# Tarekbouamer/Image-Retrieval-for-Image-Based-Localization

Measured on AMD Instinct MI355X. Metric: images/sec extract + queries/sec 1M-desc kNN, ResNet50-GeM 1024×768, higher is better.
Workload: dtype fp16

## Files before the change

### image-retrieval-for-image-based-localization_amd/cirtorch/_engine.py

```python

import contextlib
import ctypes
import os
import threading

import torch

PKG_DIR = os.path.dirname(os.path.dirname(os.path.abspath(__file__)))
LIB_PATH = os.environ.get("RR_LIB", os.path.join(PKG_DIR, "librr.so"))

RR_F32, RR_BF16, RR_F16, RR_I8 = 0, 1, 2, 3
RR_ACT_IDENTITY, RR_ACT_LEAKY = 0, 1
RR_POOL_GEM, RR_POOL_MAC, RR_POOL_SPOC = 0, 1, 2
RR_CONV_AFFINE, RR_CONV_RESIDUAL, RR_CONV_PERM32 = 1, 2, 4
RR_NHWC, RR_NCHW = 0, 1
RR_MATCH_NN, RR_MATCH_MNN, RR_MATCH_SNN, RR_MATCH_SMNN = 0, 1, 2, 3
RR_RESP_HARRIS, RR_RESP_GFTT, RR_RESP_HESSIAN, RR_RESP_DOG = 0, 1, 2, 3
RR_EPI_SAMPSON, RR_EPI_SYMMETRICAL = 0, 1
TUNE_KEYS = ("GEMM_CONFIG", "GEMM_STAGES", "GEMM_WIDE", "GEMM_ASTAT", "GEMM_XCD_MAP", "STREAM_1X1", "CONV3X3",
             "GRID_CUS", "GEMM8", "KNN_FUSED", "CONV3_PIPE", "STEM", "STREAM_XCD", "CONV3S", "WRES", "PAIR_MID",
             "WRES_RING")
globals().update(("RR_TUNE_" + name, key) for key, name in enumerate(TUNE_KEYS))
TUNE_SIZE_KEYS = {"PATCHNET_CHUNK": 32}
globals().update(("RR_TUNE_" + name, key) for name, key in TUNE_SIZE_KEYS.items())
# ... 10 lines not shown


class LaunchInfo(ctypes.Structure):
    _fields_ = [("kernel", ctypes.c_char * 32), ("variant", ctypes.c_char * 48), ("grid", ctypes.c_uint),
                ("block", ctypes.c_uint), ("nslices", ctypes.c_int), ("xmap", ctypes.c_int), ("launches", ctypes.c_int)]


class Region(ctypes.Structure):
    _fields_ = [(n, ctypes.c_uint16) for n in ("y0", "x0", "h", "w")]


_vp, _i, _ll, _f, _d, _sz = ctypes.c_void_p, ctypes.c_int, ctypes.c_longlong, ctypes.c_float, ctypes.c_double, ctypes.c_size_t
_SIGS = {
    "rr_version": ([], _i),
    "rr_build_info": ([], ctypes.c_char_p),
    "rr_last_error": ([], ctypes.c_char_p),
    "rr_device_arch": ([ctypes.c_char_p, _i], _i),
    "rr_image_to_nhwc": ([_vp, _i, _i, _i, _i, ctypes.POINTER(_f), ctypes.POINTER(_f), _i, _vp, _i, _i, _vp], _i),
    "rr_conv2d_fused": ([_vp, _vp, _vp, _vp, _vp, _vp, ctypes.POINTER(ConvDesc), _i, _i, _vp], _i),
    "rr_conv1x1_pair": ([_vp, _ll, _i, _vp, _vp, _vp, _i, _vp, _vp, _vp, _vp, _vp, _i, _f, _vp, _vp, _vp, _i, _i, _f,
                         _vp, _vp, _i, _vp], _i),
    "rr_conv3x3_pair": ([_vp, _i, _i, _i, _vp, _vp, _vp, _i, _f, _vp, _vp, _vp, _i, _f, _vp, _vp, _vp, _vp, _vp, _vp, _vp, _vp, _i, _f,
                         _vp, _vp, _vp, _i, _i, _f, _vp, _vp, _vp, _i, _vp], _i),
    "rr_pack_conv_weights": ([_vp, _i, _i, _i, _i, _i, _i, _i, _vp, _i, _vp], _i),
    "rr_stem_pack_weights": ([_vp, _i, _i, _i, _i, _vp, _i, _vp], _i),
    "rr_stem_conv_pool": ([_vp, _i, _i, _i, ctypes.POINTER(_f), ctypes.POINTER(_f), _i, _vp, _vp, _vp, _i, _f, _vp,
                           _i, _i, _i, _vp], _i),
    "rr_stem_conv_pool_u8": ([_vp, _i, _i, _i, ctypes.POINTER(_f), ctypes.POINTER(_f), _i, _vp, _vp, _vp, _i, _f,
                              _vp, _i, _i, _i, _vp], _i),
    "rr_image_to_nhwc_ragged": ([_vp, _vp, _i, _i, _i, _i, _i, ctypes.POINTER(_f), ctypes.POINTER(_f), _i, _vp, _i,
                                 _i, _vp], _i),
    "rr_stem_conv_pool_ragged": ([_vp, _vp, _i, _i, _i, _i, ctypes.POINTER(_f), ctypes.POINTER(_f), _i, _vp, _vp, _vp,
                                  _i, _f, _vp, _i, _i, _i, _vp], _i),
    "rr_pad_images": ([_vp, _vp, _i, _i, _i, _i, _i, _vp, _vp, _vp], _i),
    "rr_maxpool2d": ([_vp, _i, _i, _i, _i, _i, _i, _i, _vp, _i, _i, _i, _vp], _i),
    "rr_resize_bilinear": ([_vp, _i, _i, _i, _vp, _i, _i, _d, _d, _vp], _i),
    "rr_global_pool": ([_vp, _i, _i, _i, _i, _i, _f, _f, _vp, _i, _vp], _i),
    "rr_global_pool_pdev": ([_vp, _i, _i, _i, _i, _i, _f, _vp, _f, _vp, _i, _vp], _i),
    "rr_region_pool": ([_vp, _i, _i, _i, _i, ctypes.POINTER(Region), _i, _i, _f, _vp, _i, _f, _vp, _i, _vp], _i),
    "rr_region_aggregate": ([_vp, _i, _i, _i, _i, _f, _vp, _vp], _i),
    "rr_l2n_rows": ([_vp, _i, _i, _f, _vp, _vp], _i),
    "rr_linear_rows": ([_vp, _i, _i, _vp, _vp, _i, _vp, _vp], _i),
    "rr_head_workspace_bytes": ([_i, _i], _sz),
    "rr_whiten_workspace_bytes": ([_i, _i], _sz),
    "rr_whitenapply": ([_vp, _i, _i, _vp, _vp, _i, _vp, _vp, _sz, _vp], _i),
    "rr_head_l2n_whiten_l2n": ([_vp, _i, _i, _vp, _vp, _i, _f, _vp, _vp, _vp], _i),
# ... 192 lines not shown
```

### image-retrieval-for-image-based-localization_amd/cirtorch/_ops.py

```python

import ctypes
import os

import numpy as np
import torch

from . import _engine as E


def _st():
    return E.stream_ptr()


def _workspace(nbytes, device):
    return torch.empty(max(int(nbytes), 256), dtype=torch.uint8, device=device)


def image_to_nhwc(img, c_pad, dtype, mean=None, std=None):
    E.require_gpu(img)
    img = img.contiguous().float()
    n, c, h, w = img.shape
    out = torch.empty((n, h, w, c_pad), dtype=dtype, device=img.device)
    do = mean is not None
    m = (ctypes.c_float * 4)(*(list(mean) + [0.0] * (4 - c))[:4]) if do else (ctypes.c_float * 4)()
# ... 59 lines not shown
    E.require_gpu(x, w3, residual, w1)
    n, h, w, c = x.shape
    c_mid = w3.shape[0]
    y, z = _pair_out(out, (n, h, w, c_mid), (n, h, w, c_out), x.dtype, x.device)
    assert x.is_contiguous()
    if residual is not None:
        assert residual.shape == y.shape and residual.dtype == x.dtype and residual.is_contiguous()
        xp = wp = sp = hp = None
    else:
        xp, wp, sp, hp = proj
        E.require_gpu(xp, wp, sp, hp)
        assert xp.shape == x.shape and xp.dtype == x.dtype and xp.is_contiguous()
    E.check(E.lib().rr_conv1x1_pair(E.ptr(x), n * h * w, c, E.ptr(w3), E.ptr(scale3), E.ptr(shift3), c_mid,
                                    E.ptr(residual), E.ptr(xp), E.ptr(wp), E.ptr(sp), E.ptr(hp),
                                    E.RR_ACT_LEAKY if leaky3 else E.RR_ACT_IDENTITY, float(slope3),
                                    E.ptr(w1), E.ptr(scale1), E.ptr(shift1), c_out,
                                    E.RR_ACT_LEAKY if leaky1 else E.RR_ACT_IDENTITY, float(slope1), E.ptr(y), E.ptr(z),
                                    E.dtype_code(x.dtype), _st()), "rr_conv1x1_pair")
    return y, z


def conv3x3_pair(t1, w33, scale2, shift2, leaky2, slope2, w3, scale3, shift3, residual, leaky3, slope3,
                 w1, scale1, shift1, c_out, leaky1, slope1, proj=None, dynamic=None, conv1=None,
                 out=None):
    E.require_gpu(t1, w33, w3, residual, w1)
    n, h, w, c = t1.shape
    assert c == 64 and t1.is_contiguous() and tuple(w33.shape) == (64, 576) and tuple(w3.shape) == (256, 64)
    assert tuple(w1.shape) == (c_out, 256)
    y, z = _pair_out(out, (n, h, w, 256), (n, h, w, c_out), t1.dtype, t1.device)
    if residual is not None:
        assert residual.shape == y.shape and residual.dtype == t1.dtype and residual.is_contiguous()
        xp = wp = sp = hp = None
    else:
        xp, wp, sp, hp = proj
        E.require_gpu(xp, wp, sp, hp)
        assert tuple(xp.shape) == (n, h, w, 64) and xp.dtype == t1.dtype and xp.is_contiguous()
    act = lambda leaky: E.RR_ACT_LEAKY if leaky else E.RR_ACT_IDENTITY
    if dynamic is None:
        dynamic = os.environ.get("RR_C3PAIR_QUEUE", "1") != "0"
    queue = torch.zeros(8, dtype=torch.int32, device=t1.device) if dynamic else None
    w0, s0, h0, leaky0, slope0 = conv1 if conv1 is not None else (None, None, None, False, 0.0)
    if conv1 is not None:
        E.require_gpu(w0, s0, h0)
        assert proj is not None and tuple(w0.shape) == (64, 64)
    E.check(E.lib().rr_conv3x3_pair(E.ptr(t1), n, h, w, E.ptr(w0), E.ptr(s0), E.ptr(h0), act(leaky0), float(slope0),
                                    E.ptr(w33), E.ptr(scale2), E.ptr(shift2), act(leaky2),
                                    float(slope2), E.ptr(w3), E.ptr(scale3), E.ptr(shift3), E.ptr(residual),
                                    E.ptr(xp), E.ptr(wp), E.ptr(sp), E.ptr(hp), act(leaky3), float(slope3),
                                    E.ptr(w1), E.ptr(scale1), E.ptr(shift1), c_out, act(leaky1), float(slope1),
                                    E.ptr(y), E.ptr(z), E.ptr(queue), E.dtype_code(t1.dtype), _st()),
            "rr_conv3x3_pair")
    return y, z


def maxpool2d(x, k=3, stride=2, pad=1):
    E.require_gpu(x)
    n, h, w, c = x.shape
    ho = (h + 2 * pad - k) // stride + 1
    wo = (w + 2 * pad - k) // stride + 1
    y = torch.empty((n, ho, wo, c), dtype=x.dtype, device=x.device)
    E.check(E.lib().rr_maxpool2d(E.ptr(x), n, h, w, c, k, stride, pad, E.ptr(y), ho, wo, E.dtype_code(x.dtype),
                                 _st()), "rr_maxpool2d")
    return y


def pack_stem_weights(weight, dtype=torch.bfloat16):
    E.require_gpu(weight)
    w = weight.detach().float().contiguous()
    co, ci, kh, kw = w.shape
    out = torch.empty((co, 448), dtype=dtype, device=w.device)
    E.check(E.lib().rr_stem_pack_weights(E.ptr(w), co, ci, kh, kw, E.ptr(out), E.dtype_code(dtype), _st()),
            "rr_stem_pack_weights")
    return out

# ... 1221 lines not shown
```

### image-retrieval-for-image-based-localization_amd/cirtorch/backbones/misc.py

```python

from collections import OrderedDict

import torch
import torch.nn as nn

from .. import _ops
from ..modules.abn import ABN


class ConvStep:
    __slots__ = ("w", "kh", "kw", "stride", "pad", "c_out", "scale", "shift", "leaky", "slope", "perm")


def make_step(conv, bn, dtype, cin_pad=None, leaky_override=None):
    st = ConvStep()
    co, ci, kh, kw = conv.weight.shape
    cin_pad = cin_pad or ci
    st.perm = co % 32 == 0
    st.w = _ops.pack_conv_weights(conv.weight, cin_pad, dtype, perm32=st.perm)
    st.kh, st.kw = kh, kw
    st.stride = conv.stride[0]
    st.pad = conv.padding[0]
    st.c_out = co
    st.scale, st.shift = bn.folded()
    st.leaky, st.slope = bn.slope()
    if leaky_override is not None:
        st.leaky = leaky_override
    return st


def run_step(t, st, residual=None, out=None):
    return _ops.conv2d_fused(t, st.w, st.kh, st.kw, st.stride, st.pad, st.c_out, st.scale, st.shift,
                             residual=residual, leaky=st.leaky, slope=st.slope, perm32=st.perm, out=out)


class ResidualBlock(nn.Module):
    def __init__(self, in_channels, channels, stride=1, dilation=1, groups=1, norm_act=ABN, dropout=None):
        super().__init__()
        if len(channels) != 2 and len(channels) != 3:
            raise ValueError("channels must contain either two or three values")
        if len(channels) == 2 and groups != 1:
            raise ValueError("groups > 1 are only valid if len(channels) == 3")
        if groups != 1 or dilation != 1:
            raise NotImplementedError("grouped / dilated residual blocks are out of scope")
        self.is_bottleneck = len(channels) == 3
        self.stride = stride
# ... 64 lines not shown
```

### image-retrieval-for-image-based-localization_amd/cirtorch/backbones/resnet.py

```python

import os
import sys
from collections import OrderedDict
from functools import partial

import torch
import torch.nn as nn
import torch.nn.functional as F

from .. import _ops
from ..modules.abn import ABN
from .misc import ResidualBlock, make_step, run_step

CONV_PARAMS = ["weight"]
BN_PARAMS = ["weight", "bias", "running_mean", "running_var"]

_PRECISIONS = {"bf16": torch.bfloat16, "fp32": torch.float32, "float32": torch.float32, "bfloat16": torch.bfloat16,
               "fp16": torch.float16, "float16": torch.float16}


def try_index(scalar_or_list, i):
    try:
        return scalar_or_list[i]
    except TypeError:
# ... 94 lines not shown
        self._plan = None
        return super()._load_from_state_dict(*args, **kwargs)

    def stem_cin(self):
        return 4 if self.engine_dtype == torch.float32 else 8

    def _step(self, conv, bn, cin_pad=None, leaky_override=None):
        return make_step(conv, bn, self.engine_dtype, cin_pad=cin_pad, leaky_override=leaky_override)

    def _build_plan(self):
        dev = self.mod1.conv1.weight.device
        if dev.type != "cuda":
            raise RuntimeError("the MI355X engine runs on the GPU: call .cuda() on the model first")
        plan = {"stem": self._step(self.mod1.conv1, self.mod1.bn1, cin_pad=self.stem_cin()), "mods": []}
        plan["stem_fused"] = None
        if self.engine_dtype in (torch.bfloat16, torch.float16) and tuple(self.mod1.conv1.weight.shape) == (64, 3, 7, 7) \
                and hasattr(self.mod1, "pool1") and os.environ.get("RR_STEM_FUSED", "1") != "0":
            plan["stem_fused"] = _ops.pack_stem_weights(self.mod1.conv1.weight, self.engine_dtype)
        for mod_id in range(4):
            mod = getattr(self, "mod%d" % (mod_id + 2))
            blocks = []
            for blk in mod.children():
                blocks.append(blk.engine_plan(self.engine_dtype))
            plan["mods"].append(blocks)
        self._plan = plan
        return plan

    @staticmethod
    def _conv(t, st, residual=None, out=None):
        return run_step(t, st, residual, out)

    def _stem(self, plan, x, mean, std):
        if isinstance(x, (list, tuple)):
            live = [t for t in x if t is not None]
            if not live:
                raise ValueError("at least one image of the batch must be non-None")
            h = max(int(t.shape[-2]) for t in live)
            w = max(int(t.shape[-1]) for t in live)
            st = plan["stem"]
            if plan["stem_fused"] is not None:
                return _ops.stem_conv_pool_ragged(x, h, w, plan["stem_fused"], st.scale, st.shift, leaky=st.leaky,
                                                  slope=st.slope, mean=mean, std=std)
            t = _ops.image_to_nhwc_ragged(x, h, w, self.stem_cin(), self.engine_dtype, mean, std)
            return _ops.maxpool2d(self._conv(t, st), 3, 2, 1)
        if x.dtype == torch.uint8 and plan["stem_fused"] is None:
            x = _ops.pixels_to_unit(x)
        if plan["stem_fused"] is not None:
            st = plan["stem"]
            return _ops.stem_conv_pool(x, plan["stem_fused"], st.scale, st.shift, leaky=st.leaky, slope=st.slope,
                                       mean=mean, std=std)
        t = _ops.image_to_nhwc(x, self.stem_cin(), self.engine_dtype, mean, std)
        t = self._conv(t, plan["stem"])
        return _ops.maxpool2d(t, 3, 2, 1)

    def _blocks(self, t, flat, i0, i1, outs, pending=None):
        for i in range(i0, i1):
            mod_id, steps, proj = flat[i]
            nxt = flat[i + 1][1][0] if i + 1 < i1 else None
            pair = self._pairable(steps[-1], nxt)
            fuse_proj = pair and proj is not None and self._proj_fusable(proj)
            res = t if proj is None else (None if fuse_proj else self._conv(t, proj))
            block = pair and self._c3pairable(t, steps, nxt, fuse_proj)
            conv1 = block and fuse_proj and pending is None and self._conv1_fusable(t, steps[0])
            y = t
            for j, st in enumerate(steps[:-2] if block else steps[:-1]):
                if conv1:
                    break
                y = pending if (j == 0 and pending is not None) else self._conv(y, st)
            pending = None
            if block:
                mid, last = steps[-2], steps[-1]
                c1 = steps[0]
                t, pending = _ops.conv3x3_pair(y, mid.w, mid.scale, mid.shift, mid.leaky, mid.slope,
                                               last.w, last.scale, last.shift, res, last.leaky, last.slope,
                                               nxt.w, nxt.scale, nxt.shift, nxt.c_out, nxt.leaky, nxt.slope,
                                               proj=(t, proj.w, proj.scale, proj.shift) if fuse_proj else None,
                                               conv1=(c1.w, c1.scale, c1.shift, c1.leaky, c1.slope) if conv1 else None)
            elif pair:
                last = steps[-1]
                t, pending = _ops.conv1x1_pair(y, last.w, last.scale, last.shift, res, last.leaky, last.slope,
                                               nxt.w, nxt.scale, nxt.shift, nxt.c_out, nxt.leaky, nxt.slope,
                                               proj=(t, proj.w, proj.scale, proj.shift) if fuse_proj else None)
            else:
                t = self._conv(y, steps[-1], residual=res)
            if outs is not None and (i + 1 == len(flat) or flat[i + 1][0] != mod_id):
                outs["mod%d" % (mod_id + 2)] = t
        return t, pending

    def forward(self, x, normalize=None):
        plan = self._plan or self._build_plan()
        mean, std = normalize if normalize is not None else (None, None)
        outs = OrderedDict()
        flat = [(mod_id, steps, proj) for mod_id, blocks in enumerate(plan["mods"]) for steps, proj in blocks]
        t = self._stem(plan, x, mean, std)
        outs["mod1"] = t
        self._blocks(t, flat, 0, len(flat), outs)
        return OrderedDict((k, v.permute(0, 3, 1, 2)) for k, v in outs.items())

    @staticmethod
    def _proj_fusable(proj):
        return (proj.kh == 1 and proj.stride == 1 and proj.pad == 0 and proj.perm and proj.c_out == 256
                and proj.w.shape[1] == 64 and not proj.leaky)

    @staticmethod
    def _c3pairable(t, steps, nxt, fuse_proj):
        if len(steps) != 3 or os.environ.get("RR_C3PAIR", "1") == "0":
            return False
        mid, last = steps[1], steps[2]
        n, h, w, c = t.shape
        return (mid.kh == 3 and mid.kw == 3 and mid.stride == 1 and mid.pad == 1 and mid.perm and mid.c_out == 64
                and tuple(mid.w.shape) == (64, 576) and last.c_out == 256 and last.w.shape[1] == 64
                and nxt.c_out in ((64,) if fuse_proj else (64, 128)) and h % 4 == 0 and w % 32 == 0
                and n * h * w * 64 * 2 < 2 ** 31)

    @staticmethod
    def _conv1_fusable(t, st):
        return (os.environ.get("RR_C3PAIR_CONV1", "0") == "1" and st.kh == 1 and st.kw == 1 and st.stride == 1
                and st.pad == 0 and st.perm and st.c_out == 64 and tuple(st.w.shape) == (64, 64) and t.shape[-1] == 64)

    def _pairable(self, last, nxt):
# ... 26 lines not shown
```

### image-retrieval-for-image-based-localization_amd/cirtorch/models/GF_net.py

```python

import os
from collections import OrderedDict

import numpy as np
import torch
import torch.nn as nn

from .. import _ops
from ..algos.GF_algo import globalFeatureAlgo
from ..backbones import resnet as _resnet
from ..modules.heads.global_head import globalHead
from ..modules.pools import POOLING_LAYERS
from ..utils.parallel import PackedSequence

from ..modules.utils import OUTPUT_DIM


class Normalize:

    def __init__(self, rgb_mean=(0.485, 0.456, 0.406), rgb_std=(0.229, 0.224, 0.225)):
        self.rgb_mean = list(rgb_mean)
        self.rgb_std = list(rgb_std)


# ... 3 lines not shown
        self.augment = augment
        self.body = body
        self.ret_algo = ret_algo
        self.ret_head = ret_head
        self.meta = {}

    def _prepare_pyramid_inputs(self, img, scales):
        out = []
        for scale in scales:
            if scale == 1:
                out.append(img)
            else:
                out.append(PackedSequence([_ops.resize_bilinear(im, scale) for im in img]))
        return out

    def _normalizer(self):
        a = self.augment
        if a is None:
            return None
        if hasattr(a, "rgb_mean") and hasattr(a, "rgb_std"):
            return (list(a.rgb_mean), list(a.rgb_std))
        raise NotImplementedError("only normalising augment objects (rgb_mean/rgb_std) are supported at eval time")

    @property
    def pool(self):
        return self.ret_head.pool

    def meta_repr(self):
        tmp = "  (meta): dict( \n"
        for k in ("architecture", "local_whitening", "pooling", "regional", "whitening", "outputdim", "mean", "std"):
            if k in self.meta:
                tmp += "     %s: %s\n" % (k, self.meta[k])
        tmp += "  )\n"
        return tmp

    def forward(self, img=None, positive_img=None, negative_img=None, scales=[1], do_augmentaton=False,
                do_loss=False, do_prediction=True, **varargs):
        if do_loss:
            raise NotImplementedError("training (tuple loss) is out of scope for the MI355X engine")
        if isinstance(img, torch.Tensor) and img.dim() == 4 and len(scales) == 1:
            x = self.body(img, normalize=self._normalizer())
            ret_pred = self.ret_algo.inference(self.ret_head, x, [img.shape[-2:]] * img.shape[0]) \
                if do_prediction else None
            return OrderedDict([("ret_loss", None)]), OrderedDict([("ret_pred", ret_pred)])
        if isinstance(img, torch.Tensor) and img.dim() == 4:
            preds = []
            for scale in scales:
                if scale == 1:
                    xs = img
                else:
                    xf = _ops.pixels_to_unit(img) if img.dtype == torch.uint8 else img
                    xs = _ops.resize_bilinear(xf, scale)
                _, pred = self.forward(img=xs, scales=[1], do_prediction=True, do_loss=False)
                preds.append(pred["ret_pred"].unsqueeze(0))
            pred = torch.cat(preds, dim=0).permute(1, 2, 0)
            pred = nn.functional.avg_pool1d(pred, kernel_size=len(scales)).squeeze(-1)
            return OrderedDict([("ret_loss", None)]), OrderedDict([("ret_pred", pred)])
        if isinstance(img, torch.Tensor):
            if img.dtype == torch.uint8 and len(scales) > 1:
                img = _ops.pixels_to_unit(img)
            img = PackedSequence(list(img)) if img.dim() == 4 else PackedSequence([img])
        if len(scales) > 1:
            if img.dtype == torch.uint8:
                img = PackedSequence([_ops.pixels_to_unit(t) if t is not None else None for t in img])
            preds = []
            for im in self._prepare_pyramid_inputs(img, scales):
                _, pred = self.forward(img=im, scales=[1], do_prediction=True, do_loss=False)
                preds.append(pred["ret_pred"].unsqueeze(0))
            pred = torch.cat(preds, dim=0).permute(1, 2, 0)
            pred = nn.functional.avg_pool1d(pred, kernel_size=len(scales)).squeeze(-1)
            return OrderedDict([("ret_loss", None)]), OrderedDict([("ret_pred", pred)])

        images = list(img)
        x = self.body(images, normalize=self._normalizer())
        valid_size = [tuple(t.shape[-2:]) if t is not None else (0, 0) for t in images]
        if do_prediction:
            ret_pred = self.ret_algo.inference(self.ret_head, x, valid_size)
        else:
            ret_pred = None
        return OrderedDict([("ret_loss", None)]), OrderedDict([("ret_pred", ret_pred)])

    def extract(self, images, scales=(1,)):
        if not isinstance(images, torch.Tensor):
            images = PackedSequence(list(images))
        with torch.no_grad():
            _, pred = self.forward(img=images, scales=list(scales))
        return pred["ret_pred"]


def make_net(architecture="resnet50", pooling="gem", whitening=True, mean=None, std=None, precision="bf16",
             p=3.0, regional=False, regional_whitening=True, L=3):
    body = _resnet.__dict__[architecture](precision=precision)
    dim = OUTPUT_DIM[architecture]
    pname = {"gem": "GeM", "mac": "MAC", "spoc": "SPoC", "gemmp": "GeMmp"}[pooling.lower()]
    params = {"p": p, "eps": 1e-6} if pname in ("GeM", "GeMmp") else {}
    if regional:
        if pname == "GeMmp":
# ... 326 lines not shown
```

### image-retrieval-for-image-based-localization_amd/csrc/rr_c3pair.hip

```cpp
#include "rr_internal.h"
#include "rr_ldsdma.h"
#include "rr_epilogue.h"
#include "rr_tilewalk.h"

#ifndef C3P_IG2
#define C3P_IG2 1
#endif

namespace rr {

namespace {

template <int K>
__device__ __forceinline__ int cwswz(int row, int chunk) {
    const int f = K == 64 ? ((row >> 1) & 7) : (row & 15);
    return row * (K * 2) + ((chunk ^ f) << 4);
}

}

struct C3PairArgs {
    const bf16_t* t1;
    const bf16_t* w0;
    const float *s0, *h0;
    const bf16_t* w33;
    const float *s33, *h33;
    const bf16_t* w3;
    const float *s3, *h3;
    const bf16_t* res;
    const bf16_t* xp;
    const bf16_t* wp;
    const float *sp, *hp;
    const bf16_t* w1;
    const float *s1, *h1;
    bf16_t* y;
    bf16_t* z;
    int* queue;
    int n, h, w;
    int act2, act3, act1, act0;
    float slope2, slope3, slope1, slope0;
};

namespace {

template <int C1, bool PROJ, typename HT, bool CONV1 = false>
__global__ void __launch_bounds__(512, 1) k_c3pair(C3PairArgs a, int tiles_w, int tiles_hw, int ntiles) {
    static_assert(!CONV1 || PROJ, "conv1 in the launch: the stage's first block only");
    constexpr int TH = 4, TW = 32, TP = TH * TW, PITCH = 40;
    constexpr int NSLOT = (TH + 2) * PITCH, NP = NSLOT / 8;
    constexpr int PCW = TW + 2;
    constexpr int FN = 4;
    constexpr int K3 = 64, C3 = 256, NK3 = K3 / 32, NR3 = C3 / 32, NF1 = C1 / 16, NK1 = C3 / 32;
    static_assert(NSLOT % 8 == 0 && PITCH % 8 == 0, "row-invariant patch swizzle");
    __shared__ __attribute__((aligned(1024))) char sPatch[NSLOT * 128];
    __shared__ __attribute__((aligned(16))) char sT2[TP * 128];
    __shared__ __attribute__((aligned(16))) char sW3[C3 * K3 * 2];
    __shared__ __attribute__((aligned(16))) char sW1[C1 * C3 * 2];
    __shared__ __attribute__((aligned(16))) char sWp[PROJ ? C3 * K3 * 2 : 16];
    __shared__ __attribute__((aligned(16))) float sS3[C3], sH3[C3], sS1[C1], sH1[C1], sS2[64], sH2[64];
    __shared__ __attribute__((aligned(16))) float sSp[PROJ ? C3 : 4], sHp[PROJ ? C3 : 4];
    __shared__ __attribute__((aligned(16))) char sW0[CONV1 ? 64 * 64 * 2 : 16];
    __shared__ __attribute__((aligned(16))) float sS0[CONV1 ? 64 : 4], sH0[CONV1 ? 64 : 4];
    __shared__ int sTile[4];

    const int tid = threadIdx.x, lane = tid & 63;
    const int wave = __builtin_amdgcn_readfirstlane(tid >> 6);
    const bool role3 = wave < 4;
    const int r16 = lane & 15, kq = lane >> 4, lrow = lane >> 3, lch = lane & 7;
    const int H = a.h, W = a.w;

// ... 154 lines not shown
            sh[r] = sH2[c + r];
        }
        const bool leaky2 = a.act2 == RR_ACT_LEAKY;
#pragma unroll
        for (int j = 0; j < FN; ++j) {
            const int p = wpx * (TP / 2) + j * 16 + r16;
            float v[8];
            RR_BN_PAIR(acc[0][j], acc[1][j], sc, sh, v);
            if (leaky2) RR_LEAKY(8, v, a.slope2);
            uint4 o;
            RR_PACK8(HT, o, v);
            *reinterpret_cast<uint4*>(sT2 + p * 128 + (((4 * wc + kq) ^ (p & 7)) << 4)) = o;
        }
    };

    const int pw = wave - 4;
    const bool leaky3 = a.act3 == RR_ACT_LEAKY, leaky1 = a.act1 == RR_ACT_LEAKY;
    constexpr int NRQ = PROJ ? NK3 : NR3;
    auto strip_pixel = [&](int t, int k) __attribute__((always_inline)) {
        int img, oh0, ow0;
        tile_org(t, img, oh0, ow0);
        return ((long long)img * H + oh0 + (k >> 1)) * W + ow0 + (k & 1) * 16 + r16;
    };
    auto load_rq = [&](uint4 (&dst)[NRQ], long long p) __attribute__((always_inline)) {
        if constexpr (PROJ) {
            const bf16_t* ps = a.xp + p * K3 + 8 * kq;
#pragma unroll
            for (int kk = 0; kk < NK3; ++kk) dst[kk] = ld16_once(ps + kk * 32);
        } else {
            const bf16_t* rs = a.res + p * C3 + 8 * kq;
#pragma unroll
            for (int i2 = 0; i2 < NR3; ++i2) dst[i2] = ld16_once(rs + 32 * i2);
        }
    };
    auto pair_strip = [&](int k, long long p, const uint4 (&rv)[NRQ]) __attribute__((always_inline)) {
        uint4 bq[NK3];
        {
            const int q = k * 16 + r16;
#pragma unroll
            for (int kk = 0; kk < NK3; ++kk)
                bq[kk] = *reinterpret_cast<const uint4*>(sT2 + q * 128 + (((4 * kk + kq) ^ (q & 7)) << 4));
        }
        uint4 yq[NR3];
        constexpr int IG = C3P_IG2 ? 2 : 1;
#pragma unroll
        for (int i0 = 0; i0 < NR3; i0 += IG) {
            int abase = 0;
            asm volatile("" : "+v"(abase));
            f32x4_t acc3[IG][2], pacc[IG][2];
#pragma unroll
            for (int g = 0; g < IG; ++g)
#pragma unroll
                for (int hh = 0; hh < 2; ++hh) acc3[g][hh] = pacc[g][hh] = (f32x4_t){0.f, 0.f, 0.f, 0.f};
#pragma unroll
            for (int kk = 0; kk < NK3; ++kk)
#pragma unroll
                for (int g = 0; g < IG; ++g)
#pragma unroll
// ... 10 lines not shown
                        for (int hh = 0; hh < 2; ++hh) {
                            const uint4 av = *reinterpret_cast<const uint4*>(sWp + abase + cwswz<K3>((2 * (i0 + g) + hh) * 16 + r16, kk * 4 + kq));
                            pacc[g][hh] = H16<HT>::mfma(av, rv[kk], pacc[g][hh]);
                        }
            }
#pragma unroll
            for (int g = 0; g < IG; ++g) {
                const int i2 = i0 + g;
                const int c = 32 * i2 + 8 * kq;
                float v[8];
                RR_BN_PAIR(acc3[g][0], acc3[g][1], sS3 + c, sH3 + c, v);
                if constexpr (PROJ) {
#pragma unroll
                    for (int r = 0; r < 4; ++r) {
                        v[r] += pacc[g][0][r] * sSp[c + r] + sHp[c + r];
                        v[4 + r] += pacc[g][1][r] * sSp[c + 4 + r] + sHp[c + 4 + r];
                    }
                } else {
                    const uint4 qv = rv[i2];
                    RR_ADD_PACKED8(HT, qv, v);
                }
                if (leaky3) RR_LEAKY(8, v, a.slope3);
                RR_PACK8(HT, yq[i2], v);
                st16_once(a.y + p * C3 + c, yq[i2]);
            }
        }
        f32x4_t zacc[NF1];
        RR_ZERO(1, zacc);
#pragma unroll
        for (int kk = 0; kk < NK1; ++kk) {
            int abase = 0;
            asm volatile("" : "+v"(abase));
#pragma unroll
            for (int o = 0; o < NF1; ++o) {
                const uint4 av = *reinterpret_cast<const uint4*>(sW1 + abase + cwswz<C3>(o * 16 + r16, kk * 4 + kq));
                zacc[o] = H16<HT>::mfma(av, yq[kk], zacc[o]);
            }
        }
#pragma unroll
        for (int o2 = 0; o2 < NF1 / 2; ++o2) {
            const int c = 32 * o2 + 8 * kq;
            float v[8];
            RR_BN_PAIR(zacc[2 * o2], zacc[2 * o2 + 1], sS1 + c, sH1 + c, v);
            if (leaky1) RR_LEAKY(8, v, a.slope1);
            uint4 o;
            RR_PACK8(HT, o, v);
            st16_once(a.z + p * C1 + c, o);
// ... 39 lines not shown
                if (wpx == 0) store_t2();
                const int t2i = tile_id(s + 2);
                patch_dma(t2i, t2i >= 0);
                if (tid == 0) sTile[(s + 3) & 3] = t2i >= 0 ? fetch_tile(s + 3) : -1;
                vm_wait<0>();
            }
            lds_barrier();
        }
    } else {
        __builtin_amdgcn_s_setprio(1);
        uint4 rq[4][NRQ];
        load_rq(rq[0], strip_pixel(tile_id(0), pw));
        load_rq(rq[1], strip_pixel(tile_id(0), 4 + pw));
        lds_barrier();
        if constexpr (CONV1) lds_barrier();
        lds_barrier();
        lds_barrier();
        for (int s = 0; tile_id(s) >= 0; s += 2) {
            {
                const int t = tile_id(s);
                const bool n1 = tile_id(s + 1) >= 0;
                if (n1) load_rq(rq[2], strip_pixel(tile_id(s + 1), pw));
                if constexpr (CONV1) lds_barrier();
                pair_strip(pw, strip_pixel(t, pw), rq[0]);
                lds_barrier();
                if (n1) load_rq(rq[3], strip_pixel(tile_id(s + 1), 4 + pw));
                pair_strip(4 + pw, strip_pixel(t, 4 + pw), rq[1]);
                lds_barrier();
            }
            if (tile_id(s + 1) >= 0) {
                const int t = tile_id(s + 1);
                const bool n2 = tile_id(s + 2) >= 0;
                if (n2) load_rq(rq[0], strip_pixel(tile_id(s + 2), pw));
                if constexpr (CONV1) lds_barrier();
                pair_strip(pw, strip_pixel(t, pw), rq[2]);
                lds_barrier();
                if (n2) load_rq(rq[1], strip_pixel(tile_id(s + 2), 4 + pw));
                pair_strip(4 + pw, strip_pixel(t, 4 + pw), rq[3]);
                lds_barrier();
            }
        }
    }
}

}

}

using namespace rr;

extern "C" int rr_conv3x3_pair(const void* t1, int n, int h, int w, const void* w0, const float* scale0,
                               const float* shift0, int act0, float slope0, const void* w33, const float* scale2,
                               const float* shift2, int act2, float slope2, const void* w3, const float* scale3,
                               const float* shift3, const void* residual, const void* xp, const void* wp,
                               const float* scalep, const float* shiftp, int act3, float slope3, const void* w1,
                               const float* scale1, const float* shift1, int c_out, int act1, float slope1, void* y,
                               void* z, int* tile_queue, int dtype, void* stream) {
    if (dtype != RR_BF16 && dtype != RR_F16) return fail(RR_EINVAL, "rr_conv3x3_pair: dtype (bf16 / fp16)");
    if (!t1 || !w33 || !scale2 || !shift2 || !w3 || !scale3 || !shift3 || !w1 || !scale1 || !shift1 || !y || !z)
        return fail(RR_EINVAL, "rr_conv3x3_pair: null pointer");
    const bool proj = residual == nullptr;
    if (proj && (!xp || !wp || !scalep || !shiftp))
        return fail(RR_EINVAL, "rr_conv3x3_pair: either residual or the projection (xp, wp, scalep, shiftp)");
    if (c_out != 64 && c_out != 128) return fail(RR_EINVAL, "rr_conv3x3_pair: c_out 64 or 128");
    if (proj && c_out != 64) return fail(RR_EINVAL, "rr_conv3x3_pair: the projection form takes c_out = 64");
    const bool conv1 = w0 != nullptr;
    if (conv1 && (!proj || !scale0 || !shift0 || ((uintptr_t)w0 & 15)))
        return fail(RR_EINVAL, "rr_conv3x3_pair: conv1 in the launch (w0) needs the projection form, scale0, shift0");
    if (conv1 && act0 != RR_ACT_IDENTITY && act0 != RR_ACT_LEAKY) return fail(RR_EINVAL, "rr_conv3x3_pair: act0");
    if (n <= 0 || h <= 0 || w <= 0 || h % 4 || w % 32) return fail(RR_EINVAL, "rr_conv3x3_pair: h % 4, w % 32");
    if ((long long)n * h * w * 64 * 2 >= (1ll << 31)) return fail(RR_EINVAL, "rr_conv3x3_pair: t1 over 2 GiB (split the batch)");
    for (const void* p : {t1, w33, w3, residual, xp, wp, w1, (const void*)y, (const void*)z})
        if ((uintptr_t)p & 15) return fail(RR_EINVAL, "rr_conv3x3_pair: 16-byte alignment required");
    if ((uintptr_t)tile_queue & 3) return fail(RR_EINVAL, "rr_conv3x3_pair: tile_queue alignment");
    for (int act : {act2, act3, act1})
        if (act != RR_ACT_IDENTITY && act != RR_ACT_LEAKY) return fail(RR_EINVAL, "rr_conv3x3_pair: activation");
    C3PairArgs a;
    a.t1 = (const bf16_t*)t1; a.w33 = (const bf16_t*)w33; a.s33 = scale2; a.h33 = shift2;
    a.w3 = (const bf16_t*)w3; a.s3 = scale3; a.h3 = shift3; a.res = (const bf16_t*)residual;
    a.xp = (const bf16_t*)xp; a.wp = (const bf16_t*)wp; a.sp = scalep; a.hp = shiftp;
    a.w1 = (const bf16_t*)w1; a.s1 = scale1; a.h1 = shift1; a.y = (bf16_t*)y; a.z = (bf16_t*)z;
    a.n = n; a.h = h; a.w = w; a.act2 = act2; a.act3 = act3; a.act1 = act1;
    a.slope2 = slope2; a.slope3 = slope3; a.slope1 = slope1; a.queue = tile_queue;
    a.w0 = (const bf16_t*)w0; a.s0 = scale0; a.h0 = shift0; a.act0 = act0; a.slope0 = slope0;
    const int tiles_w = w / 32, tiles_hw = (h / 4) * tiles_w;
    const long long ntl = (long long)n * tiles_hw;
    if (ntl >= (1ll << 31)) return fail(RR_EINVAL, "rr_conv3x3_pair: too many tiles");
    const int cus = grid_cus();
    const int grid = persistent_grid8(ntl, cus);
    const dim3 g((unsigned)grid), b(512);
    hipStream_t s = as_stream(stream);
    auto go = [&](auto hv) {
        using H = decltype(hv);
        if (conv1) hipLaunchKernelGGL((k_c3pair<64, true, H, true>), g, b, 0, s, a, tiles_w, tiles_hw, (int)ntl);
        else if (proj) hipLaunchKernelGGL((k_c3pair<64, true, H>), g, b, 0, s, a, tiles_w, tiles_hw, (int)ntl);
        else if (c_out == 64) hipLaunchKernelGGL((k_c3pair<64, false, H>), g, b, 0, s, a, tiles_w, tiles_hw, (int)ntl);
        else hipLaunchKernelGGL((k_c3pair<128, false, H>), g, b, 0, s, a, tiles_w, tiles_hw, (int)ntl);
    };
    if (dtype == RR_F16) go(f16_t{});
    else go(bf16_t{});
    note_launch("k_c3pair", (unsigned)grid, 512, 0, 1, 1, "%d%s%s", c_out, proj ? ",proj" : "", conv1 ? ",conv1" : "");
    return check_launch("rr_conv3x3_pair");
}
```

### include/rr.h

```cpp
#ifndef RR_H_
#define RR_H_

#include <stddef.h>
#include <stdint.h>

#ifdef __cplusplus
extern "C" {
#endif

enum rr_dtype { RR_F32 = 0, RR_BF16 = 1, RR_F16 = 2, RR_I8 = 3 };
enum rr_act { RR_ACT_IDENTITY = 0, RR_ACT_LEAKY = 1 };
enum rr_pool_mode { RR_POOL_GEM = 0, RR_POOL_MAC = 1, RR_POOL_SPOC = 2 };
enum rr_conv_flags { RR_CONV_AFFINE = 1, RR_CONV_RESIDUAL = 2, RR_CONV_PERM32 = 4 };
enum rr_layout { RR_NHWC = 0, RR_NCHW = 1 };

#define RR_OK 0
#define RR_EINVAL -1
#define RR_EHIP -2
#define RR_ENOSPACE -3

int rr_version(void);
const char* rr_build_info(void);
const char* rr_last_error(void);
int rr_device_arch(char* buf, int buflen);
// ... 14 lines not shown
    int flags;
} rr_conv_desc;

int rr_conv2d_fused(const void* x, const void* w, const float* scale, const float* shift,
                    const void* residual, void* y, const rr_conv_desc* desc,
                    int dtype, int out_dtype, void* stream);

int rr_pack_conv_weights(const float* w, int c_out, int c_in, int kh, int kw, int c_in_pad,
                         int k_packed, int perm32, void* out, int dtype, void* stream);

int rr_conv1x1_pair(const void* x, long long p, int c_in, const void* w3, const float* scale3,
                    const float* shift3, int c_mid, const void* residual, const void* xp, const void* wp,
                    const float* scalep, const float* shiftp, int act3, float slope3, const void* w1,
                    const float* scale1, const float* shift1, int c_out, int act1, float slope1, void* y,
                    void* z, int dtype, void* stream);

int rr_conv3x3_pair(const void* t1, int n, int h, int w, const void* w0, const float* scale0,
                    const float* shift0, int act0, float slope0, const void* w33, const float* scale2,
                    const float* shift2, int act2, float slope2, const void* w3, const float* scale3,
                    const float* shift3, const void* residual, const void* xp, const void* wp,
                    const float* scalep, const float* shiftp, int act3, float slope3, const void* w1,
                    const float* scale1, const float* shift1, int c_out, int act1, float slope1, void* y,
                    void* z, int* tile_queue, int dtype, void* stream);

int rr_maxpool2d(const void* x, int n, int h, int w, int c, int k, int stride, int pad,
                 void* y, int ho, int wo, int dtype, void* stream);

int rr_stem_pack_weights(const float* w, int c_out, int c_in, int kh, int kw, void* out, int dtype, void* stream);
int rr_stem_conv_pool(const float* x, int n, int h, int w, const float* mean_host, const float* std_host,
                      int do_normalize, const void* wpk, const float* scale, const float* shift, int act,
                      float slope, void* y, int hp, int wp, int dtype, void* stream);
int rr_stem_conv_pool_u8(const unsigned char* x, int n, int h, int w, const float* mean_host,
                         const float* std_host, int do_normalize, const void* wpk, const float* scale,
                         const float* shift, int act, float slope, void* y, int hp, int wp, int dtype,
                         void* stream);

int rr_image_to_nhwc_ragged(const void* const* srcs, const int* extents, int n, int c, int h, int w, int u8,
                            const float* mean_host, const float* std_host, int do_normalize,
                            void* dst, int c_pad, int dtype, void* stream);
int rr_stem_conv_pool_ragged(const void* const* srcs, const int* extents, int n, int h, int w, int u8,
                             const float* mean_host, const float* std_host, int do_normalize, const void* wpk,
                             const float* scale, const float* shift, int act, float slope, void* y, int hp, int wp,
                             int dtype, void* stream);
int rr_pad_images(const void* const* srcs, const int* extents, int n, int c, int h, int w, int elem_bytes,
                  const void* pad_value_host, void* dst, void* stream);

// ... 223 lines not shown
```

Baseline: 5515.

## Write only stride-2 subsampled block output when next projection is strided and stage unused

When the last stage-2 block feeds a stage whose stride-2 1x1 projection is the only consumer of its full output, and that intermediate stage output is not requested, the fused conv3x3 pair kernel stores only every other pixel of y. The projection then runs as a stride-1 1x1 conv on the half-resolution tensor. Forward gains a stages filter so GF_net asks only for mod5, which lets this path trigger. This removes about three quarters of the y write traffic and the strided gather in the projection, at the cost of an extra kernel specialization and a more complex planning path.

```diff
diff --git a/image-retrieval-for-image-based-localization_amd/cirtorch/_engine.py b/image-retrieval-for-image-based-localization_amd/cirtorch/_engine.py
--- a/image-retrieval-for-image-based-localization_amd/cirtorch/_engine.py
+++ b/image-retrieval-for-image-based-localization_amd/cirtorch/_engine.py
@@ -56,6 +56,8 @@
                          _vp, _vp, _i, _vp], _i),
     "rr_conv3x3_pair": ([_vp, _i, _i, _i, _vp, _vp, _vp, _i, _f, _vp, _vp, _vp, _i, _f, _vp, _vp, _vp, _vp, _vp, _vp, _vp, _vp, _i, _f,
                          _vp, _vp, _vp, _i, _i, _f, _vp, _vp, _vp, _i, _vp], _i),
+    "rr_conv3x3_pair_s2": ([_vp, _i, _i, _i, _vp, _vp, _vp, _i, _f, _vp, _vp, _vp, _i, _f, _vp, _vp, _vp, _vp, _vp, _vp, _vp, _vp, _i, _f,
+                            _vp, _vp, _vp, _i, _i, _f, _vp, _vp, _i, _vp, _i, _vp], _i),
     "rr_pack_conv_weights": ([_vp, _i, _i, _i, _i, _i, _i, _i, _vp, _i, _vp], _i),
     "rr_stem_pack_weights": ([_vp, _i, _i, _i, _i, _vp, _i, _vp], _i),
     "rr_stem_conv_pool": ([_vp, _i, _i, _i, ctypes.POINTER(_f), ctypes.POINTER(_f), _i, _vp, _vp, _vp, _i, _f, _vp,
diff --git a/image-retrieval-for-image-based-localization_amd/cirtorch/_ops.py b/image-retrieval-for-image-based-localization_amd/cirtorch/_ops.py
--- a/image-retrieval-for-image-based-localization_amd/cirtorch/_ops.py
+++ b/image-retrieval-for-image-based-localization_amd/cirtorch/_ops.py
@@ -105,14 +105,15 @@
 
 def conv3x3_pair(t1, w33, scale2, shift2, leaky2, slope2, w3, scale3, shift3, residual, leaky3, slope3,
                  w1, scale1, shift1, c_out, leaky1, slope1, proj=None, dynamic=None, conv1=None,
-                 out=None):
+                 out=None, y_stride2=False):
     E.require_gpu(t1, w33, w3, residual, w1)
     n, h, w, c = t1.shape
     assert c == 64 and t1.is_contiguous() and tuple(w33.shape) == (64, 576) and tuple(w3.shape) == (256, 64)
     assert tuple(w1.shape) == (c_out, 256)
-    y, z = _pair_out(out, (n, h, w, 256), (n, h, w, c_out), t1.dtype, t1.device)
+    y, z = _pair_out(out, (n, h // 2, w // 2, 256) if y_stride2 else (n, h, w, 256), (n, h, w, c_out), t1.dtype,
+                     t1.device)
     if residual is not None:
-        assert residual.shape == y.shape and residual.dtype == t1.dtype and residual.is_contiguous()
+        assert tuple(residual.shape) == (n, h, w, 256) and residual.dtype == t1.dtype and residual.is_contiguous()
         xp = wp = sp = hp = None
     else:
         xp, wp, sp, hp = proj
@@ -126,13 +127,16 @@
     if conv1 is not None:
         E.require_gpu(w0, s0, h0)
         assert proj is not None and tuple(w0.shape) == (64, 64)
-    E.check(E.lib().rr_conv3x3_pair(E.ptr(t1), n, h, w, E.ptr(w0), E.ptr(s0), E.ptr(h0), act(leaky0), float(slope0),
-                                    E.ptr(w33), E.ptr(scale2), E.ptr(shift2), act(leaky2),
-                                    float(slope2), E.ptr(w3), E.ptr(scale3), E.ptr(shift3), E.ptr(residual),
-                                    E.ptr(xp), E.ptr(wp), E.ptr(sp), E.ptr(hp), act(leaky3), float(slope3),
-                                    E.ptr(w1), E.ptr(scale1), E.ptr(shift1), c_out, act(leaky1), float(slope1),
-                                    E.ptr(y), E.ptr(z), E.ptr(queue), E.dtype_code(t1.dtype), _st()),
-            "rr_conv3x3_pair")
+    args = (E.ptr(t1), n, h, w, E.ptr(w0), E.ptr(s0), E.ptr(h0), act(leaky0), float(slope0),
+            E.ptr(w33), E.ptr(scale2), E.ptr(shift2), act(leaky2),
+            float(slope2), E.ptr(w3), E.ptr(scale3), E.ptr(shift3), E.ptr(residual),
+            E.ptr(xp), E.ptr(wp), E.ptr(sp), E.ptr(hp), act(leaky3), float(slope3),
+            E.ptr(w1), E.ptr(scale1), E.ptr(shift1), c_out, act(leaky1), float(slope1), E.ptr(y), E.ptr(z))
+    tail = (E.ptr(queue), E.dtype_code(t1.dtype), _st())
+    if y_stride2:
+        E.check(E.lib().rr_conv3x3_pair_s2(*args, 1, *tail), "rr_conv3x3_pair_s2")
+    else:
+        E.check(E.lib().rr_conv3x3_pair(*args, *tail), "rr_conv3x3_pair")
     return y, z
 
 
diff --git a/image-retrieval-for-image-based-localization_amd/cirtorch/backbones/misc.py b/image-retrieval-for-image-based-localization_amd/cirtorch/backbones/misc.py
--- a/image-retrieval-for-image-based-localization_amd/cirtorch/backbones/misc.py
+++ b/image-retrieval-for-image-based-localization_amd/cirtorch/backbones/misc.py
@@ -9,7 +9,7 @@
 
 
 class ConvStep:
-    __slots__ = ("w", "kh", "kw", "stride", "pad", "c_out", "scale", "shift", "leaky", "slope", "perm")
+    __slots__ = ("w", "kh", "kw", "stride", "pad", "c_out", "scale", "shift", "leaky", "slope", "perm", "s1")
 
 
 def make_step(conv, bn, dtype, cin_pad=None, leaky_override=None):
@@ -22,6 +22,7 @@
     st.stride = conv.stride[0]
     st.pad = conv.padding[0]
     st.c_out = co
+    st.s1 = None
     st.scale, st.shift = bn.folded()
     st.leaky, st.slope = bn.slope()
     if leaky_override is not None:
diff --git a/image-retrieval-for-image-based-localization_amd/cirtorch/backbones/resnet.py b/image-retrieval-for-image-based-localization_amd/cirtorch/backbones/resnet.py
--- a/image-retrieval-for-image-based-localization_amd/cirtorch/backbones/resnet.py
+++ b/image-retrieval-for-image-based-localization_amd/cirtorch/backbones/resnet.py
@@ -1,4 +1,5 @@
 
+import copy
 import os
 import sys
 from collections import OrderedDict
@@ -140,6 +141,10 @@
             blocks = []
             for blk in mod.children():
                 blocks.append(blk.engine_plan(self.engine_dtype))
+                proj = blocks[-1][1]
+                if proj is not None and proj.kh == 1 and proj.kw == 1 and proj.stride == 2 and proj.pad == 0:
+                    proj.s1 = copy.copy(proj)
+                    proj.s1.stride = 1
             plan["mods"].append(blocks)
         self._plan = plan
         return plan
@@ -171,14 +176,20 @@
         t = self._conv(t, plan["stem"])
         return _ops.maxpool2d(t, 3, 2, 1)
 
-    def _blocks(self, t, flat, i0, i1, outs, pending=None):
+    def _blocks(self, t, flat, i0, i1, outs, pending=None, want=None):
+        half = False
         for i in range(i0, i1):
             mod_id, steps, proj = flat[i]
             nxt = flat[i + 1][1][0] if i + 1 < i1 else None
             pair = self._pairable(steps[-1], nxt)
             fuse_proj = pair and proj is not None and self._proj_fusable(proj)
-            res = t if proj is None else (None if fuse_proj else self._conv(t, proj))
-            block = pair and self._c3pairable(t, steps, nxt, fuse_proj)
+            if half:
+                assert proj.s1 is not None and pending is not None and not fuse_proj
+                res = self._conv(t, proj.s1)
+            else:
+                res = t if proj is None else (None if fuse_proj else self._conv(t, proj))
+            block = pair and not half and self._c3pairable(t, steps, nxt, fuse_proj)
+            half = False
             conv1 = block and fuse_proj and pending is None and self._conv1_fusable(t, steps[0])
             y = t
             for j, st in enumerate(steps[:-2] if block else steps[:-1]):
@@ -189,11 +200,14 @@
             if block:
                 mid, last = steps[-2], steps[-1]
                 c1 = steps[0]
+                half = (want is not None and "mod%d" % (mod_id + 2) not in want and flat[i + 1][0] != mod_id
+                        and self._y_stride2(proj, nxt, flat[i + 1][2]))
                 t, pending = _ops.conv3x3_pair(y, mid.w, mid.scale, mid.shift, mid.leaky, mid.slope,
                                                last.w, last.scale, last.shift, res, last.leaky, last.slope,
                                                nxt.w, nxt.scale, nxt.shift, nxt.c_out, nxt.leaky, nxt.slope,
                                                proj=(t, proj.w, proj.scale, proj.shift) if fuse_proj else None,
-                                               conv1=(c1.w, c1.scale, c1.shift, c1.leaky, c1.slope) if conv1 else None)
+                                               conv1=(c1.w, c1.scale, c1.shift, c1.leaky, c1.slope) if conv1 else None,
+                                               y_stride2=half)
             elif pair:
                 last = steps[-1]
                 t, pending = _ops.conv1x1_pair(y, last.w, last.scale, last.shift, res, last.leaky, last.slope,
@@ -202,18 +216,34 @@
             else:
                 t = self._conv(y, steps[-1], residual=res)
             if outs is not None and (i + 1 == len(flat) or flat[i + 1][0] != mod_id):
-                outs["mod%d" % (mod_id + 2)] = t
+                name = "mod%d" % (mod_id + 2)
+                if want is None or name in want:
+                    outs[name] = t
         return t, pending
 
-    def forward(self, x, normalize=None):
+    STAGES = ("mod1", "mod2", "mod3", "mod4", "mod5")
+
+    def forward(self, x, normalize=None, stages=None):
+        want = None
+        if stages is not None:
+            want = set([stages] if isinstance(stages, str) else stages)
+            unknown = sorted(want - set(self.STAGES), key=str)
+            if unknown:
+                raise ValueError("unknown stage name(s) %s: expected names out of %s" % (unknown, list(self.STAGES)))
         plan = self._plan or self._build_plan()
         mean, std = normalize if normalize is not None else (None, None)
         outs = OrderedDict()
         flat = [(mod_id, steps, proj) for mod_id, blocks in enumerate(plan["mods"]) for steps, proj in blocks]
         t = self._stem(plan, x, mean, std)
-        outs["mod1"] = t
-        self._blocks(t, flat, 0, len(flat), outs)
+        if want is None or "mod1" in want:
+            outs["mod1"] = t
+        self._blocks(t, flat, 0, len(flat), outs, want=want)
         return OrderedDict((k, v.permute(0, 3, 1, 2)) for k, v in outs.items())
+
+    @staticmethod
+    def _y_stride2(proj, nxt, nxt_proj):
+        return (os.environ.get("RR_C3PAIR_YS2", "1") != "0" and proj is None and nxt.c_out == 128
+                and nxt_proj is not None and nxt_proj.s1 is not None)
 
     @staticmethod
     def _proj_fusable(proj):
diff --git a/image-retrieval-for-image-based-localization_amd/cirtorch/models/GF_net.py b/image-retrieval-for-image-based-localization_amd/cirtorch/models/GF_net.py
--- a/image-retrieval-for-image-based-localization_amd/cirtorch/models/GF_net.py
+++ b/image-retrieval-for-image-based-localization_amd/cirtorch/models/GF_net.py
@@ -49,6 +49,9 @@
             return (list(a.rgb_mean), list(a.rgb_std))
         raise NotImplementedError("only normalising augment objects (rgb_mean/rgb_std) are supported at eval time")
 
+    def _body_stages(self):
+        return {"stages": ("mod5",)} if isinstance(self.body, _resnet.ResNet) else {}
+
     @property
     def pool(self):
         return self.ret_head.pool
@@ -66,7 +69,7 @@
         if do_loss:
             raise NotImplementedError("training (tuple loss) is out of scope for the MI355X engine")
         if isinstance(img, torch.Tensor) and img.dim() == 4 and len(scales) == 1:
-            x = self.body(img, normalize=self._normalizer())
+            x = self.body(img, normalize=self._normalizer(), **self._body_stages())
             ret_pred = self.ret_algo.inference(self.ret_head, x, [img.shape[-2:]] * img.shape[0]) \
                 if do_prediction else None
             return OrderedDict([("ret_loss", None)]), OrderedDict([("ret_pred", ret_pred)])
@@ -99,7 +102,7 @@
             return OrderedDict([("ret_loss", None)]), OrderedDict([("ret_pred", pred)])
 
         images = list(img)
-        x = self.body(images, normalize=self._normalizer())
+        x = self.body(images, normalize=self._normalizer(), **self._body_stages())
         valid_size = [tuple(t.shape[-2:]) if t is not None else (0, 0) for t in images]
         if do_prediction:
             ret_pred = self.ret_algo.inference(self.ret_head, x, valid_size)
diff --git a/image-retrieval-for-image-based-localization_amd/csrc/rr_c3pair.hip b/image-retrieval-for-image-based-localization_amd/csrc/rr_c3pair.hip
--- a/image-retrieval-for-image-based-localization_amd/csrc/rr_c3pair.hip
+++ b/image-retrieval-for-image-based-localization_amd/csrc/rr_c3pair.hip
@@ -43,9 +43,25 @@
 
 namespace {
 
-template <int C1, bool PROJ, typename HT, bool CONV1 = false>
+template <typename T>
+struct YStride2 {};
+template <typename T>
+struct C3PairHalf {
+    using type = T;
+    static constexpr bool ys2 = false;
+};
+template <typename T>
+struct C3PairHalf<YStride2<T>> {
+    using type = T;
+    static constexpr bool ys2 = true;
+};
+
+template <int C1, bool PROJ, typename HS, bool CONV1 = false>
 __global__ void __launch_bounds__(512, 1) k_c3pair(C3PairArgs a, int tiles_w, int tiles_hw, int ntiles) {
+    using HT = typename C3PairHalf<HS>::type;
+    constexpr bool YS2 = C3PairHalf<HS>::ys2;
     static_assert(!CONV1 || PROJ, "conv1 in the launch: the stage's first block only");
+    static_assert(!YS2 || (!PROJ && C1 == 128), "stride-2 y: the stage's last block only");
     constexpr int TH = 4, TW = 32, TP = TH * TW, PITCH = 40;
     constexpr int NSLOT = (TH + 2) * PITCH, NP = NSLOT / 8;
     constexpr int PCW = TW + 2;
@@ -246,6 +262,11 @@
         tile_org(t, img, oh0, ow0);
         return ((long long)img * H + oh0 + (k >> 1)) * W + ow0 + (k & 1) * 16 + r16;
     };
+    auto strip_pixel_s2 = [&](int t, int k) __attribute__((always_inline)) {
+        int img, oh0, ow0;
+        tile_org(t, img, oh0, ow0);
+        return ((long long)img * (H >> 1) + ((oh0 + (k >> 1)) >> 1)) * (W >> 1) + ((ow0 + (k & 1) * 16 + r16) >> 1);
+    };
     auto load_rq = [&](uint4 (&dst)[NRQ], long long p) __attribute__((always_inline)) {
         if constexpr (PROJ) {
             const bf16_t* ps = a.xp + p * K3 + 8 * kq;
@@ -257,7 +278,10 @@
             for (int i2 = 0; i2 < NR3; ++i2) dst[i2] = ld16_once(rs + 32 * i2);
         }
     };
-    auto pair_strip = [&](int k, long long p, const uint4 (&rv)[NRQ]) __attribute__((always_inline)) {
+    auto pair_strip = [&](int t, int k, long long p, const uint4 (&rv)[NRQ]) __attribute__((always_inline)) {
+        bf16_t* ys = nullptr;
+        if constexpr (YS2)
+            if (!(k & 2) && !(r16 & 1)) ys = a.y + strip_pixel_s2(t, k) * C3 + 8 * kq;
         uint4 bq[NK3];
         {
             const int q = k * 16 + r16;
@@ -314,7 +338,11 @@
                 }
                 if (leaky3) RR_LEAKY(8, v, a.slope3);
                 RR_PACK8(HT, yq[i2], v);
-                st16_once(a.y + p * C3 + c, yq[i2]);
+                if constexpr (YS2) {
+                    if (ys) st16_once(ys + 32 * i2, yq[i2]);
+                } else {
+                    st16_once(a.y + p * C3 + c, yq[i2]);
+                }
             }
         }
         f32x4_t zacc[NF1];
@@ -400,10 +428,10 @@
                 const bool n1 = tile_id(s + 1) >= 0;
                 if (n1) load_rq(rq[2], strip_pixel(tile_id(s + 1), pw));
                 if constexpr (CONV1) lds_barrier();
-                pair_strip(pw, strip_pixel(t, pw), rq[0]);
+                pair_strip(t, pw, strip_pixel(t, pw), rq[0]);
                 lds_barrier();
                 if (n1) load_rq(rq[3], strip_pixel(tile_id(s + 1), 4 + pw));
-                pair_strip(4 + pw, strip_pixel(t, 4 + pw), rq[1]);
+                pair_strip(t, 4 + pw, strip_pixel(t, 4 + pw), rq[1]);
                 lds_barrier();
             }
             if (tile_id(s + 1) >= 0) {
@@ -411,10 +439,10 @@
                 const bool n2 = tile_id(s + 2) >= 0;
                 if (n2) load_rq(rq[0], strip_pixel(tile_id(s + 2), pw));
                 if constexpr (CONV1) lds_barrier();
-                pair_strip(pw, strip_pixel(t, pw), rq[2]);
+                pair_strip(t, pw, strip_pixel(t, pw), rq[2]);
                 lds_barrier();
                 if (n2) load_rq(rq[1], strip_pixel(tile_id(s + 2), 4 + pw));
-                pair_strip(4 + pw, strip_pixel(t, 4 + pw), rq[3]);
+                pair_strip(t, 4 + pw, strip_pixel(t, 4 + pw), rq[3]);
                 lds_barrier();
             }
         }
@@ -434,6 +462,18 @@
                                const float* scalep, const float* shiftp, int act3, float slope3, const void* w1,
                                const float* scale1, const float* shift1, int c_out, int act1, float slope1, void* y,
                                void* z, int* tile_queue, int dtype, void* stream) {
+    return rr_conv3x3_pair_s2(t1, n, h, w, w0, scale0, shift0, act0, slope0, w33, scale2, shift2, act2, slope2, w3,
+                              scale3, shift3, residual, xp, wp, scalep, shiftp, act3, slope3, w1, scale1, shift1,
+                              c_out, act1, slope1, y, z, 0, tile_queue, dtype, stream);
+}
+
+extern "C" int rr_conv3x3_pair_s2(const void* t1, int n, int h, int w, const void* w0, const float* scale0,
+                                  const float* shift0, int act0, float slope0, const void* w33, const float* scale2,
+                                  const float* shift2, int act2, float slope2, const void* w3, const float* scale3,
+                                  const float* shift3, const void* residual, const void* xp, const void* wp,
+                                  const float* scalep, const float* shiftp, int act3, float slope3, const void* w1,
+                                  const float* scale1, const float* shift1, int c_out, int act1, float slope1,
+                                  void* y, void* z, int y_stride2, int* tile_queue, int dtype, void* stream) {
     if (dtype != RR_BF16 && dtype != RR_F16) return fail(RR_EINVAL, "rr_conv3x3_pair: dtype (bf16 / fp16)");
     if (!t1 || !w33 || !scale2 || !shift2 || !w3 || !scale3 || !shift3 || !w1 || !scale1 || !shift1 || !y || !z)
         return fail(RR_EINVAL, "rr_conv3x3_pair: null pointer");
@@ -446,6 +486,9 @@
     if (conv1 && (!proj || !scale0 || !shift0 || ((uintptr_t)w0 & 15)))
         return fail(RR_EINVAL, "rr_conv3x3_pair: conv1 in the launch (w0) needs the projection form, scale0, shift0");
     if (conv1 && act0 != RR_ACT_IDENTITY && act0 != RR_ACT_LEAKY) return fail(RR_EINVAL, "rr_conv3x3_pair: act0");
+    if (y_stride2 && (proj || conv1 || c_out != 128))
+        return fail(RR_EINVAL, "rr_conv3x3_pair_s2: y_stride2 takes the residual form with c_out = 128 (no projection, "
+                               "no conv1 in the launch)");
     if (n <= 0 || h <= 0 || w <= 0 || h % 4 || w % 32) return fail(RR_EINVAL, "rr_conv3x3_pair: h % 4, w % 32");
     if ((long long)n * h * w * 64 * 2 >= (1ll << 31)) return fail(RR_EINVAL, "rr_conv3x3_pair: t1 over 2 GiB (split the batch)");
     for (const void* p : {t1, w33, w3, residual, xp, wp, w1, (const void*)y, (const void*)z})
@@ -473,10 +516,12 @@
         if (conv1) hipLaunchKernelGGL((k_c3pair<64, true, H, true>), g, b, 0, s, a, tiles_w, tiles_hw, (int)ntl);
         else if (proj) hipLaunchKernelGGL((k_c3pair<64, true, H>), g, b, 0, s, a, tiles_w, tiles_hw, (int)ntl);
         else if (c_out == 64) hipLaunchKernelGGL((k_c3pair<64, false, H>), g, b, 0, s, a, tiles_w, tiles_hw, (int)ntl);
-        else hipLaunchKernelGGL((k_c3pair<128, false, H>), g, b, 0, s, a, tiles_w, tiles_hw, (int)ntl);
+        else if (!y_stride2) hipLaunchKernelGGL((k_c3pair<128, false, H>), g, b, 0, s, a, tiles_w, tiles_hw, (int)ntl);
+        else hipLaunchKernelGGL((k_c3pair<128, false, YStride2<H>>), g, b, 0, s, a, tiles_w, tiles_hw, (int)ntl);
     };
     if (dtype == RR_F16) go(f16_t{});
     else go(bf16_t{});
-    note_launch("k_c3pair", (unsigned)grid, 512, 0, 1, 1, "%d%s%s", c_out, proj ? ",proj" : "", conv1 ? ",conv1" : "");
+    note_launch("k_c3pair", (unsigned)grid, 512, 0, 1, 1, "%d%s%s%s", c_out, proj ? ",proj" : "", conv1 ? ",conv1" : "",
+                y_stride2 ? ",ys2" : "");
     return check_launch("rr_conv3x3_pair");
 }
diff --git a/include/rr.h b/include/rr.h
--- a/include/rr.h
+++ b/include/rr.h
@@ -60,6 +60,14 @@
                     const float* scalep, const float* shiftp, int act3, float slope3, const void* w1,
                     const float* scale1, const float* shift1, int c_out, int act1, float slope1, void* y,
                     void* z, int* tile_queue, int dtype, void* stream);
+
+int rr_conv3x3_pair_s2(const void* t1, int n, int h, int w, const void* w0, const float* scale0,
+                       const float* shift0, int act0, float slope0, const void* w33, const float* scale2,
+                       const float* shift2, int act2, float slope2, const void* w3, const float* scale3,
+                       const float* shift3, const void* residual, const void* xp, const void* wp,
+                       const float* scalep, const float* shiftp, int act3, float slope3, const void* w1,
+                       const float* scale1, const float* shift1, int c_out, int act1, float slope1, void* y,
+                       void* z, int y_stride2, int* tile_queue, int dtype, void* stream);
 
 int rr_maxpool2d(const void* x, int n, int h, int w, int c, int k, int stride, int pad,
                  void* y, int ho, int wo, int dtype, void* stream);
```

New measurement: 5544, median of 6. No clear change (+0.5%).
